# davlee1972/upscale_video

Measured on AMD Instinct MI355X. Metric: frames/sec 1080p->2x Compact (SRVGGNetCompact per-frame SR hot path), higher is better.
Workload: dtype f16 operands / f32 accumulate; 1 GPU; 2x_compact_1080p; tile_size=960, frames_per_call=1

## Files before the change

### upscale_video_amd/csrc/uva_api.hip

```cpp
#include "../../include/uva.h"
#include "uva_denoise.hip.h"
#include "uva_denoise16.hip.h"
#include "uva_generic.hip.h"
#include "uva_kernels.hip.h"
#include "uva_model.h"
#include "uva_pixfmt.h"
#include "uva_plan.h"
#include "uva_repeat.h"
#include "uva_crop.h"
#include "uva_resize.h"
#include "uva_png.hip.h"
#include "uva_wino.h"
#include "uva_sub5.h"
#include "uva_sub10.h"

namespace uva {
int png_read_bgr(const uint8_t* file, size_t len, uint8_t* out, size_t cap, int* h_out, int* w_out, std::string& err);
int png_read_bgr16(const uint8_t* file, size_t len, uint16_t* out, size_t cap, int* h_out, int* w_out, std::string& err);
int zlib_decompress_exact(const uint8_t* in, size_t n, uint8_t* out, size_t out_len, std::string& err);
}

#include <hip/hip_runtime.h>

#include <algorithm>
// ... 264 lines not shown
template <typename T>
int upload(T** dst, const void* src, size_t bytes, hipStream_t st)
{
    HIP_TRY(hipMalloc((void**)dst, bytes));
    HIP_TRY(hipMemcpyAsync(*dst, src, bytes, hipMemcpyHostToDevice, st));
    return 0;
}


template <int NF, int MODE, int R>
int launch_conv_t(uva_net* n, const ConvArgs& a)
{
    const size_t lds = conv_lds_bytes<NF>(MODE == 0 ? 0 : R);
    auto kfn = conv3x3_kernel<NF, MODE, R>;
    if (!n->attr_set[MODE]) {
        HIP_TRY(hipFuncSetAttribute((const void*)kfn, hipFuncAttributeMaxDynamicSharedMemorySize, (int)lds));
        n->attr_set[MODE] = true;
    }
    const int per_cu = NF == 24 ? 2 : 1;
    const int grid = std::max(8, (n->ncu / 8) * 8) * per_cu;
    hipLaunchKernelGGL(kfn, dim3(grid), dim3(256), lds, n->stream, a);
    HIP_TRY(hipGetLastError());
    return 0;
}

template <int ABL>
int launch_trunk64_t(uva_net* n, const ConvArgs& a)
{
    const size_t lds = trunk_lds_bytes<64>();
    auto kfn = trunk_kernel<64, ABL>;
    constexpr int SLOT = 3 + (ABL == 0 ? 0 : ABL == 1 ? 1 : ABL == 2 ? 2 : 3);
    if (!n->attr_set[SLOT]) {
        HIP_TRY(hipFuncSetAttribute((const void*)kfn, hipFuncAttributeMaxDynamicSharedMemorySize, (int)lds));
        n->attr_set[SLOT] = true;
    }
    const int grid = std::max(8, (n->ncu / 8) * 8);
    hipLaunchKernelGGL(kfn, dim3(grid), dim3(512), lds, n->stream, a);
    HIP_TRY(hipGetLastError());
    return 0;
}

int launch_trunk64(uva_net* n, const ConvArgs& a, int ablate = 0)
{
#ifdef UVA_INSTRUMENT
    if (ablate == 1) return launch_trunk64_t<1>(n, a);
    if (ablate == 2) return launch_trunk64_t<2>(n, a);
    if (ablate == 4) return launch_trunk64_t<4>(n, a);
#endif
    (void)ablate;
    return launch_trunk64_t<0>(n, a);
}

template <int NF>
int launch_conv_nf(uva_net* n, int mode, int r, const ConvArgs& a)
{
    if (mode == 0) return launch_conv_t<NF, 0, 1>(n, a);
    if (mode == 1) {
        if (r == 1) return launch_conv_t<NF, 1, 1>(n, a);
        if (r == 2) return launch_conv_t<NF, 1, 2>(n, a);
        if (r == 4) return launch_conv_t<NF, 1, 4>(n, a);
    } else {
        if (r == 1) return launch_conv_t<NF, 2, 1>(n, a);
        if (r == 2) return launch_conv_t<NF, 2, 2>(n, a);
        if (r == 4) return launch_conv_t<NF, 2, 4>(n, a);
    }
    return fail("no kernel for this scale");
}

int launch_conv(uva_net* n, int mode, const ConvArgs& a)
{
    if (n->g.nf == 64) return launch_conv_nf<64>(n, mode, n->g.scale, a);
    if (n->g.nf == 24) return launch_conv_nf<24>(n, mode, n->g.scale, a);
    return fail("no kernel for this trunk width");
}

bool has_tail64(const uva_net* n) { return n->g.nf == 64 && (n->g.scale == 2 || n->g.scale == 4) && n->layers.back().wpk16; }

int launch_tail_u8(uva_net* n, const Workspace* ws, ConvArgs ca, bool u16 = false)
{
    if (has_tail64(n)) {
        const bool x4 = n->g.scale == 4;
        size_t lds;
        void (*kfn)(ConvArgs);
        if (u16) {
            lds = x4 ? tail4_lds_bytes<64, uint16_t>() : tail_lds_bytes<64, uint16_t>();
            kfn = x4 ? tail4_kernel<64, uint16_t> : tail_kernel<64, 2, uint16_t>;
        } else {
            lds = x4 ? tail4_lds_bytes<64>() : tail_lds_bytes<64>();
            kfn = x4 ? tail4_kernel<64, uint8_t> : tail_kernel<64, 2, uint8_t>;
        }
        const int slot = u16 ? 10 : 7;
        if (!n->attr_set[slot]) {
            HIP_TRY(hipFuncSetAttribute((const void*)kfn, hipFuncAttributeMaxDynamicSharedMemorySize, (int)lds));
            n->attr_set[slot] = true;
        }
        const int grid = std::max(8, (n->ncu / 8) * 8);
        const int per_launch = 8 * (2 * (grid / 8)) * ((TAIL_SCHED_MAX - TRUNK_LOOKAHEAD) / 2 - 1);
        ca.sched4 = ws->d_sched4;
        ca.wpk = n->layers.back().wpk16;
        for (int base = 0; base < ws->ntiles4; base += per_launch) {
            ca.tile_base = base;
            ca.ntiles = std::min(per_launch, ws->ntiles4 - base);
            ca.tiles_per_xcd = (ca.ntiles + 7) / 8;
            hipLaunchKernelGGL(kfn, dim3(grid), dim3(512), lds, n->stream, ca);
            HIP_TRY(hipGetLastError());
        }
        return 0;
    }
    if (u16) return fail("the 16-bit route has no tail for this net");
    return launch_conv(n, 1, ca);
}

int launch_trunk(uva_net* n, const Workspace* ws, ConvArgs ca, int ablate = 0)
{
    if (n->g.nf == 64) {
        const int grid = std::max(8, (n->ncu / 8) * 8);
        const int per_launch = 8 * (2 * (grid / 8)) * ((TRUNK_SCHED_MAX - TRUNK_LOOKAHEAD) / 2 - 1);
        ca.sched4 = ws->d_sched4;
        for (int base = 0; base < ws->ntiles4; base += per_launch) {
            ca.tile_base = base;
            ca.ntiles = std::min(per_launch, ws->ntiles4 - base);
            ca.tiles_per_xcd = (ca.ntiles + 7) / 8;
            if (launch_trunk64(n, ca, ablate)) return 1;
        }
        return 0;
    }
    ca.ntiles = ws->ntiles;
    ca.tiles_per_xcd = (ws->ntiles + 7) / 8;
    return launch_conv(n, 0, ca);
}

int launch_trunk2(uva_net* n, const Workspace* ws, const Trunk2Args& a)
{
    const size_t lds = trunk2_lds_bytes<64>();
    auto kfn = trunk2_kernel<64>;
    if (!n->attr_set[8]) {
        HIP_TRY(hipFuncSetAttribute((const void*)kfn, hipFuncAttributeMaxDynamicSharedMemorySize, (int)lds));
        n->attr_set[8] = true;
    }
    hipLaunchKernelGGL(kfn, dim3(ws->grid2), dim3(512), lds, n->stream, a);
    HIP_TRY(hipGetLastError());
    return 0;
}

int launch_trunkw(uva_net* n, const Workspace* ws, TrunkwArgs& a, int i, bool in_negated = false, bool carry_out = false)
{
    for (int k = 0; k < 2; ++k) {
        a.wpk[k] = n->layers[i + k].wpk_w;
        a.bias[k] = n->act16 ? n->layers[i + k].bias_w : n->layers[i + k].bias;
        a.slope[k] = n->layers[i + k].slope;
    }
    if (in_negated) a.wpk[0] = n->layers[i].wpk_wn;
    const int act = !n->act16 ? TW_ACT_F32 : (n->layers[i + 1].flip_w && !carry_out) ? TW_ACT_F16_FLIP : TW_ACT_F16;
    HIP_TRY(launch_trunkw_kernel(n->stream, ws->grid2, a, act));
    return 0;
}

int launch_sub5(uva_net* n, Workspace* ws, const void* src, size_t src_stride, void* dst, size_t dst_stride,
                unsigned long long* dbg = nullptr, int dbg_part = -1)
{
    if (ws->sub5_unfit) return 2;
    if (!ws->d_rows5) {
        std::vector<uint4> rows;
        std::vector<int> nrows;
        ws->grid5 = std::max(8, (n->ncu / 8) * 8);
        std::string err;
        const int rc = build_sub5_rows(ws->h, ws->w, ws->grid5, rows, nrows, &ws->max_rows5, err);
        if (rc == 1) return fail(err);
        if (rc) {
            ws->sub5_unfit = true;
            return 2;
        }
        char* d_mid = nullptr;
        uint4* d_rows = nullptr;
        int* d_nrows = nullptr;
        hipError_t e = hipMalloc((void**)&d_mid, (size_t)ws->h * ws->w * S5_MIDB);
        if (e == hipSuccess) e = hipMalloc((void**)&d_rows, rows.size() * sizeof(uint4));
        if (e == hipSuccess) e = hipMalloc((void**)&d_nrows, nrows.size() * sizeof(int));
        if (e == hipSuccess) e = hipMemcpyAsync(d_rows, rows.data(), rows.size() * sizeof(uint4), hipMemcpyHostToDevice, n->stream);
        if (e == hipSuccess) e = hipMemcpyAsync(d_nrows, nrows.data(), nrows.size() * sizeof(int), hipMemcpyHostToDevice, n->stream);
        if (e == hipSuccess) e = hipStreamSynchronize(n->stream);
        if (e != hipSuccess) {
            if (d_mid) (void)hipFree(d_mid);
            if (d_rows) (void)hipFree(d_rows);
            if (d_nrows) (void)hipFree(d_nrows);
            return fail(std::string("sub5 workspace: ") + hipGetErrorString(e));
        }
        ws->d_mid5 = d_mid; ws->d_rows5 = d_rows; ws->d_nrows5 = d_nrows;
    }
    for (int part = 0; part < 2; ++part) {
        Sub5Args a;
        std::memset(&a, 0, sizeof a);
        a.src = (const uint8_t*)src; a.src_stride = src_stride;
        a.dst = (uint8_t*)dst; a.dst_stride = dst_stride;
        a.mid = ws->d_mid5;
        a.h = ws->h; a.w = ws->w;
        a.rows = ws->d_rows5; a.nrows = ws->d_nrows5; a.max_rows = ws->max_rows5;
        a.dbg = part == dbg_part ? dbg : nullptr;
        for (int i = 0; i < S5_NL; ++i) {
            a.wpk[i] = n->layers[S5_NL * part + i].wpk_s10;
            a.bias[i] = n->layers[S5_NL * part + i].bias_s10;
            a.slope[i] = n->layers[S5_NL * part + i].slope;
        }
        HIP_TRY(launch_sub5_kernel(n->stream, ws->grid5, a, part));
    }
    return 0;
}

int ensure_sub10_rows(uva_net* n, Workspace* ws, int frames)
{
    if (ws->sub10_unfit || frames < 1 || frames > ws->sub10_max_batch) return 2;
    const int bi = frames - 1;
    if (!ws->d_rows10[bi]) {
        std::vector<uint4> rows;
        std::vector<int> nrows;
        ws->grid10 = std::max(8, (n->ncu / 8) * 8);
        std::string err;
        const int rc = build_sub10_rows(ws->h, ws->w, frames, ws->grid10, rows, nrows, &ws->max_rows10[bi], err);
        if (rc == 1) return fail(err);
        if (rc) {
            if (frames == 1) ws->sub10_unfit = true;
            ws->sub10_max_batch = frames - 1;
            return 2;
        }
        uint4* d_rows = nullptr;
        int* d_nrows = nullptr;
        hipError_t e = hipMalloc((void**)&d_rows, rows.size() * sizeof(uint4));
        if (e == hipSuccess) e = hipMalloc((void**)&d_nrows, nrows.size() * sizeof(int));
        if (e == hipSuccess) e = hipMemcpyAsync(d_rows, rows.data(), rows.size() * sizeof(uint4), hipMemcpyHostToDevice, n->stream);
        if (e == hipSuccess) e = hipMemcpyAsync(d_nrows, nrows.data(), nrows.size() * sizeof(int), hipMemcpyHostToDevice, n->stream);
        if (e == hipSuccess) e = hipStreamSynchronize(n->stream);
        if (e != hipSuccess) {
            if (d_rows) (void)hipFree(d_rows);
            if (d_nrows) (void)hipFree(d_nrows);
            return fail(std::string("sub10 row table: ") + hipGetErrorString(e));
        }
        ws->d_rows10[bi] = d_rows;
        ws->d_nrows10[bi] = d_nrows;
    }
    return 0;
}

int launch_sub10(uva_net* n, Workspace* ws, const void* const* srcs, size_t src_stride, void* const* dsts, size_t dst_stride, int frames,
                 unsigned long long* dbg = nullptr)
{
    if (const int rc = ensure_sub10_rows(n, ws, frames)) return rc;
    const int bi = frames - 1;
    Sub10Args a;
    std::memset(&a, 0, sizeof a);
    for (int f = 0; f < S10_MAXB; ++f) {
        a.src[f] = (const uint8_t*)srcs[std::min(f, frames - 1)];
        a.dst[f] = (uint8_t*)dsts[std::min(f, frames - 1)];
    }
    a.src_stride = src_stride;
    a.dst_stride = dst_stride;
    a.h = ws->h; a.w = ws->w;
    a.rows = ws->d_rows10[bi]; a.nrows = ws->d_nrows10[bi]; a.max_rows = ws->max_rows10[bi];
    a.dbg = dbg;
    for (int i = 0; i < S10_NL; ++i) {
        a.wpk[i] = n->layers[i].wpk_s10;
        a.bias[i] = n->layers[i].bias_s10;
        a.slope[i] = n->layers[i].slope;
    }
    HIP_TRY(launch_sub10_kernel(n->stream, ws->grid10, a));
    return 0;
}
int launch_sub10(uva_net* n, Workspace* ws, const void* src, size_t src_stride, void* dst, size_t dst_stride, unsigned long long* dbg = nullptr)
{
    return launch_sub10(n, ws, &src, src_stride, &dst, dst_stride, 1, dbg);
}

bool is_sub10_net(const uva_net* n)
{
    return !n->generic && n->g.nf == 24 && n->g.scale == 1 && (int)n->g.convs.size() == S10_NL;
}

int launch_pair24(uva_net* n, const ConvArgs& a)
{
    const size_t lds = pair24_lds_bytes();
    if (!n->attr_set[9]) {
        HIP_TRY(hipFuncSetAttribute((const void*)pair24_kernel, hipFuncAttributeMaxDynamicSharedMemorySize, (int)lds));
        n->attr_set[9] = true;
    }
    const int grid = std::max(8, (n->ncu / 8) * 8) * 2;
    hipLaunchKernelGGL(pair24_kernel, dim3(grid), dim3(256), lds, n->stream, a);
    HIP_TRY(hipGetLastError());
    return 0;
}

int launch_head(uva_net* n, bool f32, const HeadArgs& a, bool u16 = false)
{
    if (u16) {
        if (n->g.nf != 64 || !a.sink) return fail("the 16-bit route has no head for this net");
        const dim3 grid(std::min(a.ntiles, n->ncu * HEADP_WG_PER_CU)), block(256);
        hipLaunchKernelGGL((headp_kernel<64, 2>), grid, block, headp_lds_bytes<64>(), n->stream, a);
        HIP_TRY(hipGetLastError());
        return 0;
    }
    const char* const hp = uva::debug_env("UVA_HEAD_PERSIST");
    const bool persist = !hp || std::atoi(hp) != 0;
    if (persist && a.sink) {
        const dim3 grid(std::min(a.ntiles, n->ncu * HEADP_WG_PER_CU)), block(256);
        if (n->g.nf == 64) {
            const size_t lds = headp_lds_bytes<64>();
            if (f32) hipLaunchKernelGGL((headp_kernel<64, 1>), grid, block, lds, n->stream, a);
            else hipLaunchKernelGGL((headp_kernel<64, 0>), grid, block, lds, n->stream, a);
        } else {
// ... 3323 lines not shown
```

### upscale_video_amd/csrc/uva_wino.h

```cpp
#pragma once
#include <hip/hip_runtime.h>
#include <stdint.h>

#include "uva_plan.h"

namespace uva {

struct TrunkwArgs {
    const char* in_act;
    char* out_act;
    const void* wpk[2];
    const float* bias[2];
    const float* slope[2];
    const Trunk2Step* steps;
    const int* nsteps;
    int max_steps;
    _Float16* sink;
    unsigned long long* dbg;
};

enum { TW_ACT_F32 = 0, TW_ACT_F16 = 1, TW_ACT_F16_FLIP = 2 };

hipError_t launch_trunkw_kernel(hipStream_t stream, int grid, const TrunkwArgs& a, int act);

}
```

### upscale_video_amd/csrc/uva_wino.hip

```cpp
#include <atomic>

#include "uva_wino.hip.h"

namespace uva {

template <int ACT>
static hipError_t launch_act(hipStream_t stream, int grid, const TrunkwArgs& a)
{
    auto kfn = trunkw_kernel<64, ACT>;
    static std::atomic<bool> attr_done[64];
    int dev = 0;
    hipError_t e = hipGetDevice(&dev);
    if (e != hipSuccess) return e;
    if (dev < 0 || dev >= 64 || !attr_done[dev].load(std::memory_order_acquire)) {
        e = hipFuncSetAttribute((const void*)kfn, hipFuncAttributeMaxDynamicSharedMemorySize, (int)TW_LDS_BYTES);
        if (e != hipSuccess) return e;
        if (dev >= 0 && dev < 64) attr_done[dev].store(true, std::memory_order_release);
    }
    hipLaunchKernelGGL(kfn, dim3(grid), dim3(512), TW_LDS_BYTES, stream, a);
    return hipGetLastError();
}

hipError_t launch_trunkw_kernel(hipStream_t stream, int grid, const TrunkwArgs& a, int act)
{
    switch (act) {
    case TW_ACT_F32: return launch_act<TW_ACT_F32>(stream, grid, a);
    case TW_ACT_F16: return launch_act<TW_ACT_F16>(stream, grid, a);
    case TW_ACT_F16_FLIP: return launch_act<TW_ACT_F16_FLIP>(stream, grid, a);
    }
    return hipErrorInvalidValue;
}

}
```

### upscale_video_amd/csrc/uva_wino.hip.h

```cpp
#pragma once
#include <type_traits>

#include "uva_devutil.hip.h"
#include "uva_wino.h"

namespace uva {

constexpr int TW_AROWB = 4 * 2 * 16 * 64;
constexpr int TW_BROWB = 4 * 2 * 15 * 64;
constexpr int TW_AROWS = 6, TW_BROWS = 10;
constexpr int TW_RAWROWB = 34 * 128;
constexpr int TW_RAWSLOTB = 4 * TW_RAWROWB;
constexpr int TW_RAW_PIECES = TW_RAWSLOTB / 1024;
constexpr int TW_ARING = 0;
constexpr int TW_BRING = TW_ARING + TW_AROWS * TW_AROWB;
constexpr int TW_RAW = TW_BRING + TW_BROWS * TW_BROWB;
constexpr int TW_PRM = TW_RAW + 2 * TW_RAWSLOTB;
constexpr int TW_FLAGS_OFF = TW_PRM + 2 * PARAM_LDS + 64;
constexpr int TW_LDS_BYTES = TW_FLAGS_OFF + 16;
static_assert(TW_RAW_PIECES == 17 && TW_RAWSLOTB % 1024 == 0, "raw slot = whole LDS-DMA pieces");
static_assert(TW_LDS_BYTES <= 160 * 1024, "trunkw kernel LDS budget");
static_assert(TW_RAW % 128 == 0 && TW_RAWROWB % 128 == 0, "raw pixel records are 128-byte aligned (the octet XOR flips address bits 4..6)");


__device__ __forceinline__ unsigned tw_piece_const(int i, int wave, int lane)
{
    const int q = (4 * i + wave) * 64 + lane;
    const int r = q / 272, u = q - r * 272;
    const int rec = u >> 3, sl = u & 7;
    const int par = rec >= 17 ? 1 : 0, h = rec - 17 * par;
    return (unsigned)((r << 13) | ((2 * h + par) * 128 + ((sl ^ (h & 7)) << 4)));
}

__device__ __forceinline__ unsigned dpp_row_shl1(unsigned v)
{
    return (unsigned)__builtin_amdgcn_mov_dpp((int)v, 0x101, 0xf, 0xf, true);
}
__device__ __forceinline__ unsigned pk_add_f16(unsigned a, unsigned b)
{
    return __builtin_bit_cast(unsigned, (half2v)(__builtin_bit_cast(half2v, a) + __builtin_bit_cast(half2v, b)));
}

#define TW_PRIO_K 2
#define TW_PRIO_E 0
#define TW_PRIO_KA TW_PRIO_K
#define TW_PRIO_EA TW_PRIO_E
#define TW_PRIO_KB TW_PRIO_K
#define TW_PRIO_EB TW_PRIO_E

#ifdef UVA_INSTRUMENT
#define TW_STAMP(k) do { if (stamp) a.dbg[16 * it + 8 * grp + (k)] = __builtin_amdgcn_s_memtime(); } while (0)
#else
#define TW_STAMP(k) do { } while (0)
#endif

template <int NF, int ACT>
__global__ __launch_bounds__(512, 2) UVA_NO_PK_F32 void trunkw_kernel(TrunkwArgs a)
{
    static_assert(NF == 64, "written for 64 features");
    constexpr int PIXB = 128;
    constexpr int TW_PFF = 12;
    constexpr int TW_PFF_B = 6;
    constexpr int TW_RAW_F0 = 4, TW_RAW_GAP = 12, TW_RAW_STRIDE = 3;
    constexpr int TW_DMA_PIECES = 5;
    constexpr int PFF_A = TW_PFF;

    extern __shared__ __attribute__((aligned(16))) char smem[];
    const unsigned lds0 = lds_offset(smem);
    float* const prm_all = (float*)(smem + TW_PRM);

    const int wave8 = __builtin_amdgcn_readfirstlane(threadIdx.x >> 6);
    const int grp = wave8 >> 2;
    const int wave = wave8 & 3;
    const int lane = threadIdx.x & 63;

#ifdef UVA_INSTRUMENT
    const unsigned long long t_entry = __builtin_amdgcn_s_memtime();
#endif
    const Trunk2Step* const steps = a.steps + (size_t)blockIdx.x * (a.max_steps + TW_PAD_STEPS);
    auto load_a = [&](int g) __attribute__((always_inline)) { return scalar_load16(&steps[g].a); };
    auto load_b = [&](int g) __attribute__((always_inline)) { return scalar_load16(&steps[g].b); };
    const uint4 e_first = load_a(0), e_second = load_a(1);
    const int nsteps = __builtin_amdgcn_readfirstlane(a.nsteps[blockIdx.x]);
    if (nsteps <= 0) return;
#ifdef UVA_INSTRUMENT
    const bool stamp = a.dbg != nullptr && blockIdx.x == 0 && (threadIdx.x & 255) == 0;
    if (stamp && grp == 0) a.dbg[16 * (nsteps + 2)] = t_entry;
#endif

    float prm_b = 0.f, prm_s = 0.f;
    if (wave == 0) {
        prm_b = (grp ? a.bias[1] : a.bias[0])[lane];
        prm_s = (grp ? a.slope[1] : a.slope[0])[lane];
    }
    half8 w[24];
    {
        const half8* wp = (const half8*)(grp ? a.wpk[1] : a.wpk[0]);
#pragma unroll
        for (int i = 0; i < 24; ++i) w[i] = wp[(i * 4 + wave) * 64 + lane];
    }
    unsigned dma_pc2[3];
#pragma unroll
    for (int i = 0; i < 3; ++i)
        dma_pc2[i] = tw_piece_const(2 * i, wave, lane) | (2 * i + 1 < 5 ? tw_piece_const(2 * i + 1, wave, lane) << 16 : 0u);
    auto issue_rows = [&](const uint4 e, int slot, auto i0c, auto i1c) __attribute__((always_inline)) {
        constexpr int I0 = decltype(i0c)::value, I1 = decltype(i1c)::value;
        const unsigned ey = __builtin_amdgcn_readfirstlane(e.y);
        const unsigned lo = __builtin_amdgcn_readfirstlane(e.x), hi = ey & 0xffu;
        const char* base = a.in_act + (((unsigned long long)hi << 32) | lo);
        const int pitch = __builtin_amdgcn_readfirstlane(e.z) & 0xffffff;
        const unsigned fadd = ((ey >> 27) & 1u) ? (unsigned)__builtin_amdgcn_readfirstlane(e.w) : 0u;
#pragma unroll
        for (int i = I0; i < I1; ++i) {
            if (4 * i + wave >= TW_RAW_PIECES) continue;
            const unsigned pc = (dma_pc2[i >> 1] >> (16 * (i & 1))) & 0xffffu;
            unsigned off = __umul24(pc >> 13, (unsigned)pitch) + (pc & 0x1fffu);
            if (fadd) off += (pc & 0x1800u) ? fadd : 0u;
            glds16_s(base, off, lds0 + TW_RAW + slot * TW_RAWSLOTB + (4 * i + wave) * 1024);
        }
    };

    auto vlane_of = [](int l) __attribute__((always_inline)) { const int p_ = l & 15, o_ = l >> 4; return (unsigned)(p_ * 64 + ((o_ ^ ((p_ >> 1) & 3)) << 4)); };

    const unsigned vlane_c = vlane_of(lane);
    const unsigned t_lo = (unsigned)((lane & 15) * PIXB + (((lane >> 4) ^ (lane & 7)) << 4));
    const unsigned t_hi = (unsigned)(((lane & 15) + 1) * PIXB + (((lane >> 4) ^ (((lane & 15) + 1) & 7)) << 4));
    auto transform_row = [&](const char* rrow, int pos) __attribute__((always_inline)) {
        const unsigned a_lo = t_lo, a_hi = t_hi;
        char* const vrow = smem + TW_ARING + pos * TW_AROWB + vlane_c;
        half8 d[2][4];
#pragma unroll
        for (int t = 0; t < 2; ++t) {
            d[t][0] = *(const half8*)(rrow + (a_lo ^ (t ? 64u : 0u)));
            d[t][1] = *(const half8*)(rrow + (a_lo ^ (t ? 64u : 0u)) + 17 * PIXB);
            d[t][2] = *(const half8*)(rrow + (a_hi ^ (t ? 64u : 0u)));
            d[t][3] = *(const half8*)(rrow + (a_hi ^ (t ? 64u : 0u)) + 17 * PIXB);
        }
#pragma unroll
        for (int t = 0; t < 2; ++t) {
            *(half8*)(vrow + 0 * 2048 + t * 1024) = pk_sub(d[t][0], d[t][2]);
            *(half8*)(vrow + 1 * 2048 + t * 1024) = d[t][1] + d[t][2];
            *(half8*)(vrow + 2 * 2048 + t * 1024) = pk_sub(d[t][2], d[t][1]);
            *(half8*)(vrow + 3 * 2048 + t * 1024) = pk_sub(d[t][1], d[t][3]);
        }
    };

    auto transform_half = [&](const char* rrow, int pos, int t) __attribute__((always_inline)) {
        const unsigned a_lo = t_lo ^ (t ? 64u : 0u), a_hi = t_hi ^ (t ? 64u : 0u);
        char* const vrow = smem + TW_ARING + pos * TW_AROWB + vlane_c + t * 1024;
        const half8 d0 = *(const half8*)(rrow + a_lo), d1 = *(const half8*)(rrow + a_lo + 17 * PIXB);
        const half8 d2 = *(const half8*)(rrow + a_hi), d3 = *(const half8*)(rrow + a_hi + 17 * PIXB);
        *(half8*)(vrow + 0 * 2048) = pk_sub(d0, d2);
        *(half8*)(vrow + 1 * 2048) = d1 + d2;
        *(half8*)(vrow + 2 * 2048) = pk_sub(d2, d1);
        *(half8*)(vrow + 3 * 2048) = pk_sub(d1, d3);
    };

    auto transform_rows = [&](int slot, int pos0) __attribute__((always_inline)) {
        int pos = pos0 + wave;
        pos = pos >= TW_AROWS ? pos - TW_AROWS : pos;
        transform_row(smem + TW_RAW + slot * TW_RAWSLOTB + wave * TW_RAWROWB, pos);
    };

    const bool six = (__builtin_amdgcn_readfirstlane(e_first.y) >> 25) & 1u;
    if (grp == 0) {
        issue_rows(e_first, 0, std::integral_constant<int, 0>{}, std::integral_constant<int, 5>{});
        issue_rows(e_second, 1, std::integral_constant<int, 0>{}, std::integral_constant<int, 5>{});
        if (six && wave < 2) {
            const unsigned lo = __builtin_amdgcn_readfirstlane(e_first.x), hi = __builtin_amdgcn_readfirstlane(e_first.y) & 0xffu;
            const int pitch = __builtin_amdgcn_readfirstlane(e_first.z) & 0xffffff;
            const char* base = a.in_act + (((unsigned long long)hi << 32) | lo) - (size_t)(2 - wave) * pitch;
#pragma unroll
            for (int i = 0; i < 5; ++i) {
                int q = i * 64 + lane;
                q = q < 272 ? q : 271;
                const int rec = q >> 3, sl = q & 7, par = rec >= 17 ? 1 : 0, hh = rec - 17 * par;
                glds16_s(base, (unsigned)((2 * hh + par) * 128 + ((sl ^ (hh & 7)) << 4)), lds0 + TW_BRING + wave * 5120 + i * 1024);
            }
        }
#pragma unroll
        for (int i = 0; i < 24; ++i) asm volatile("" : "+v"(w[i]));
        asm volatile("s_waitcnt vmcnt(0)" ::: "memory");
    }
    if (wave == 0) {
        float* prm = prm_all + grp * (PARAM_LDS / 4);
        prm[lane] = prm_b;
        prm[64 + lane] = prm_s;
        prm[128 + lane] = prm_s <= 1.f ? __builtin_inff() : -__builtin_inff();
    }
    group_barrier();
    if (grp == 1) {
        transform_rows(0, 2);
        if (six && wave < 2) transform_row(smem + TW_BRING + wave * 5120, wave);
    }
    group_barrier();

    const float* const bias_lds = prm_all + grp * (PARAM_LDS / 4);
    const float* const prm_lds = bias_lds + 64;
    const f32x4 zero4 = {0.f, 0.f, 0.f, 0.f};
    const f32x4 bias4 = *(const f32x4*)(bias_lds + 16 * wave + 4 * (lane >> 4));
    const f32x4 s4 = *(const f32x4*)(prm_lds + 16 * wave + 4 * (lane >> 4));
    const f32x4 i4 = *(const f32x4*)(prm_lds + 64 + 16 * wave + 4 * (lane >> 4));

    f32x4 acc[4][4];
    [[maybe_unused]] auto prefetch = [&](auto ring_tag, int base_pos, auto& pre) __attribute__((always_inline)) {
        constexpr bool BR = decltype(ring_tag)::value;
        constexpr int ROWB = BR ? TW_BROWB : TW_AROWB;
        constexpr int PFF = BR ? TW_PFF_B : PFF_A;
        static_assert(PFF <= 8, "the fragments read ahead of the barrier are window row 0's");
        const unsigned r0 = vlane_c + (unsigned)((BR ? TW_BRING : TW_ARING) + base_pos * ROWB);
#pragma unroll
        for (int f = 0; f < PFF; ++f) pre[f] = *(const half8*)(smem + r0 + (f & 3) * (ROWB / 4) + ((f >> 2) & 1) * (ROWB / 8));
    };
    auto kloop = [&](auto ring_tag, int base_pos, auto&& slice, auto&& hook, [[maybe_unused]] const auto& pre) __attribute__((always_inline)) {
        constexpr bool BR = decltype(ring_tag)::value;
        constexpr int INR = 0;
        constexpr int ROWB = BR ? TW_BROWB : TW_AROWB, NROWS = BR ? TW_BROWS : TW_AROWS;
        constexpr int JS = ROWB / 4, CS = ROWB / 8;
        constexpr int PFF = BR ? TW_PFF_B : PFF_A;
        constexpr int NFRAG = 48, RQ = PFF + 1;
        unsigned radr[6];
        const unsigned vlane = vlane_c;
#pragma unroll
        for (int R = 0; R < 6; ++R) {
            int pos = base_pos + R;
            pos = pos >= NROWS ? pos - NROWS : pos;
            radr[R] = vlane + (unsigned)((BR ? TW_BRING : TW_ARING) + pos * ROWB);
        }
        auto read_f = [&](int f) __attribute__((always_inline)) -> half8 {
            const int R = f >> 3, ch = (f >> 2) & 1, j = f & 3;
            return *(const half8*)(smem + radr[R] + j * JS + ch * CS);
        };
        half8 bq[RQ];
        __builtin_amdgcn_sched_barrier(0);
#pragma unroll
        for (int f = 0; f < PFF; ++f) {
            if constexpr (BR) bq[f] = pre[f];
            else bq[f] = read_f(f);
        }
        __builtin_amdgcn_sched_barrier(0);
        static_for<NFRAG>([&](auto fc) __attribute__((always_inline)) {
            constexpr int f = decltype(fc)::value;
            if constexpr (f + PFF < NFRAG) bq[(f + PFF) % RQ] = read_f(f + PFF);
            constexpr int R = f >> 3, ch = (f >> 2) & 1, j = f & 3;
            const half8 b = bq[f % RQ];
            static_for<4>([&](auto nc) __attribute__((always_inline)) {
                constexpr int n = decltype(nc)::value, dy = R - n;
                if constexpr (dy >= 0 && dy <= 2) {
                    constexpr bool first = dy == 0 && ch == 0;
                    acc[n][j] = __builtin_amdgcn_mfma_f32_16x16x32_f16(w[(j * 3 + dy) * 2 + ch], b, first ? (j == 1 ? bias4 : zero4) : acc[n][j], 0, 0, 0);
                }
            });
            if constexpr (R >= 3 && R - 3 < INR) slice(std::integral_constant<int, R - 3>{}, std::integral_constant<int, (f & 7)>{});
            hook(fc);
            __builtin_amdgcn_sched_barrier(0);
        });
    };

    struct RowSt {
        f32x2 u, v;
        unsigned x0, x1, y0, y1;
        unsigned t[4], q[8];
    };
    f32x2 neg1 = {-1.f, -1.f};
    asm volatile("" : "+v"(neg1));
    auto fin_sum = [&](RowSt& st, int n, int hh) __attribute__((always_inline)) {
        const f32x2 m0 = {acc[n][0][2 * hh], acc[n][0][2 * hh + 1]}, m1 = {acc[n][1][2 * hh], acc[n][1][2 * hh + 1]};
        const f32x2 m2 = {acc[n][2][2 * hh], acc[n][2][2 * hh + 1]}, m3 = {acc[n][3][2 * hh], acc[n][3][2 * hh + 1]};
        st.u = (m0 + m1) + m2;
        st.v = __builtin_elementwise_fma(m3, neg1, __builtin_elementwise_fma(m2, neg1, m1));
    };
    const half2v s16v[2] = {half2v{(_Float16)s4[0], (_Float16)s4[1]}, half2v{(_Float16)s4[2], (_Float16)s4[3]}};
    auto fin_act = [&](RowSt& st, int hh) __attribute__((always_inline)) {
        if constexpr (ACT != TW_ACT_F32) {
            const half2v hu = __builtin_convertvector(st.u, half2v), hv = __builtin_convertvector(st.v, half2v);
            const half2v mu = hu * s16v[hh], mv = hv * s16v[hh];
            const unsigned xu = __builtin_bit_cast(unsigned, __builtin_elementwise_max(hu, mu));
            const unsigned xv = __builtin_bit_cast(unsigned, __builtin_elementwise_max(hv, mv));
            if (hh == 0) { st.x0 = xu; st.y0 = xv; } else { st.x1 = xu; st.y1 = xv; }
            return;
        }
        const f32x2 sl = {s4[2 * hh], s4[2 * hh + 1]};
        const f32x2 us = st.u * sl, vs = st.v * sl;
        const f32x2 pu = {__builtin_amdgcn_fmed3f(st.u[0], us[0], i4[2 * hh]), __builtin_amdgcn_fmed3f(st.u[1], us[1], i4[2 * hh + 1])};
        const f32x2 pv = {__builtin_amdgcn_fmed3f(st.v[0], vs[0], i4[2 * hh]), __builtin_amdgcn_fmed3f(st.v[1], vs[1], i4[2 * hh + 1])};
        const unsigned xu = __builtin_bit_cast(unsigned, __builtin_convertvector(pu, half2v));
        const unsigned xv = __builtin_bit_cast(unsigned, __builtin_convertvector(pv, half2v));
        if (hh == 0) { st.x0 = xu; st.y0 = xv; } else { st.x1 = xu; st.y1 = xv; }
    };

    const int niter = nsteps + 2;
    __builtin_amdgcn_s_waitcnt(0x0f70);
    RowSt st2[2];
    if (grp == 0) {
        uint4 e_own = load_a(0);
        int a6 = 0;
        int b10 = 0;
        const int cg = lane >> 4, p = lane & 15;
        const int oo = 2 * (wave & 1) + (cg >> 1);
        const unsigned wlane = p < 15 ? (unsigned)(TW_BRING + (2 * (cg & 1)) * (TW_BROWB / 4) + (wave >> 1) * (TW_BROWB / 8) + p * 64 +
                                                    ((oo ^ ((p >> 1) & 3)) << 4))
                                      : (unsigned)(TW_FLAGS_OFF - 64 + 16 * cg);
        const unsigned w64 = (unsigned)(TW_BRING + (wave >> 1) * (TW_BROWB / 8) + p * 64 + ((oo ^ ((p >> 1) & 3)) << 4) + 8 * (cg & 1));
        const unsigned wrow = p < 15 ? (unsigned)TW_BROWB : 0u;
        const unsigned wj = p < 15 ? (unsigned)(TW_BROWB / 4) : 0u;
        half8 pre[PFF_A];
        for (int it = 0; it < niter; ++it) {
            TW_STAMP(0);
            const unsigned ey = __builtin_amdgcn_readfirstlane(e_own.y);
            int rmask = 15, b10w = b10;
            bool in0 = true, in1 = true, edge = false;
            auto set_step = [&](const unsigned eyv, const int b10v) __attribute__((always_inline)) {
                const int c_lo = (eyv >> 12) & 63, c_hi = (eyv >> 18) & 63;
                rmask = (eyv >> 8) & 15;
                const int pm = ((eyv >> 27) & 1u) ? (p & 7) : p;
                in0 = 2 * pm >= c_lo && 2 * pm < c_hi;
                in1 = 2 * pm + 1 >= c_lo && 2 * pm + 1 < c_hi;
                edge = rmask != 15 || c_lo != 0 || c_hi != 32;
                b10w = b10v;
            };
            auto slice = [&](RowSt& st, auto edge_tag, auto nc, auto kc) __attribute__((always_inline)) {
                constexpr int n = decltype(nc)::value, k = decltype(kc)::value;
                if constexpr (k == 0) fin_sum(st, n, 0);
                else if constexpr (k == 1) fin_act(st, 0);
                else if constexpr (k == 2) fin_sum(st, n, 1);
                else if constexpr (k == 3) fin_act(st, 1);
                else if constexpr (k == 4) {
                    if constexpr (decltype(edge_tag)::value) {
                        const bool rin = (rmask >> n) & 1;
                        const unsigned k0 = (rin && in0) ? 0xffffffffu : 0u, k1 = (rin && in1) ? 0xffffffffu : 0u;
                        st.x0 &= k0; st.x1 &= k0;
                        st.y0 &= k1; st.y1 &= k1;
                    }
                    st.t[0] = dpp_row_shl1(st.x0); st.t[1] = dpp_row_shl1(st.x1);
                    st.t[2] = dpp_row_shl1(st.y0); st.t[3] = dpp_row_shl1(st.y1);
                } else if constexpr (k == 5) {
                    st.q[0] = pk_sub_f16(st.x0, st.t[0]); st.q[1] = pk_sub_f16(st.x1, st.t[1]);
                    st.q[2] = pk_add_f16(st.y0, st.t[0]); st.q[3] = pk_add_f16(st.y1, st.t[1]);
                    st.q[4] = pk_sub_f16(st.t[0], st.y0); st.q[5] = pk_sub_f16(st.t[1], st.y1);
                    st.q[6] = pk_sub_f16(st.y0, st.t[2]); st.q[7] = pk_sub_f16(st.y1, st.t[3]);
                } else if constexpr (k == 6) {
                    int pos = b10w + n;
                    pos = pos >= TW_BROWS ? pos - TW_BROWS : pos;
                    if (p < 15) {
                        char* const w0 = smem + w64 + (unsigned)pos * TW_BROWB;
#pragma unroll
                        for (int j = 0; j < 4; ++j) *(uint2*)(w0 + j * (TW_BROWB / 4)) = make_uint2(st.q[2 * j], st.q[2 * j + 1]);
                    }
                } else if constexpr (k == 7) {
                } else if constexpr (k == 8) {
                    const auto s02a = __builtin_amdgcn_permlane16_swap(st.q[0], st.q[4], false, false);
                    const auto s02b = __builtin_amdgcn_permlane16_swap(st.q[1], st.q[5], false, false);
                    const auto s13a = __builtin_amdgcn_permlane16_swap(st.q[2], st.q[6], false, false);
                    const auto s13b = __builtin_amdgcn_permlane16_swap(st.q[3], st.q[7], false, false);
                    st.q[0] = s02a[0]; st.q[1] = s02b[0]; st.q[2] = s02a[1]; st.q[3] = s02b[1];
                    st.q[4] = s13a[0]; st.q[5] = s13b[0]; st.q[6] = s13a[1]; st.q[7] = s13b[1];
                } else {
                    int pos = b10w + n;
                    pos = pos >= TW_BROWS ? pos - TW_BROWS : pos;
                    char* const w0 = smem + wlane + (unsigned)pos * wrow;
                    *(uint4*)w0 = make_uint4(st.q[0], st.q[1], st.q[2], st.q[3]);
                    *(uint4*)(w0 + wj) = make_uint4(st.q[4], st.q[5], st.q[6], st.q[7]);
                }
            };
            set_step(ey, b10);
            if (it < nsteps) {
                __builtin_amdgcn_s_setprio(TW_PRIO_KA);
                auto no_hook = [](auto) __attribute__((always_inline)) {};
                kloop(std::false_type{}, a6, [&](auto nc, auto kc) __attribute__((always_inline)) { slice(st2[0], std::false_type{}, nc, kc); }, no_hook, pre);
                __builtin_amdgcn_s_setprio(TW_PRIO_EA);
            }
            TW_STAMP(1);
            group_barrier();
            TW_STAMP(2);
            if (it < nsteps) {
                auto rest = [&](auto edge_tag) __attribute__((always_inline)) {
                    static_for<2>([&](auto rc) __attribute__((always_inline)) {
                        static_for<8>([&](auto kc) __attribute__((always_inline)) {
                            slice(st2[0], edge_tag, std::integral_constant<int, 2 * decltype(rc)::value>{}, kc);
                            slice(st2[1], edge_tag, std::integral_constant<int, 2 * decltype(rc)::value + 1>{}, kc);
                        });
                    });
                };
                if (edge) rest(std::true_type{}); else rest(std::false_type{});
            }
            e_own = load_a(it + 1 < nsteps ? it + 1 : nsteps - 1);
            TW_STAMP(3);
            a6 = a6 + 4 >= TW_AROWS ? a6 + 4 - TW_AROWS : a6 + 4;
            group_barrier();
            b10 = b10 + 4 >= TW_BROWS ? b10 + 4 - TW_BROWS : b10 + 4;
        }
    } else {
        int a6 = 0, b10 = 0;
        uint4 e_k = make_uint4(0, 0, 0, 0), e_3 = make_uint4(0, 0, 0, 0);
        const int cg = lane >> 4, p = lane & 15;
        const int col = 2 * p + (cg & 1);
        const unsigned olane = (unsigned)(col * PIXB + 32 * wave + 16 * (cg >> 1));
        char* const sink = (char*)a.sink + lane * PIXB;
        const unsigned flip0 = (s4[0] > 1.f ? 0x8000u : 0u) | (s4[1] > 1.f ? 0x80000000u : 0u);
        const unsigned flip1 = (s4[2] > 1.f ? 0x8000u : 0u) | (s4[3] > 1.f ? 0x80000000u : 0u);
        auto make_slice = [&](const uint4 e) __attribute__((always_inline)) {
            const unsigned ey = __builtin_amdgcn_readfirstlane(e.y), lo = __builtin_amdgcn_readfirstlane(e.x);
            const size_t off = ((unsigned long long)(ey & 0xffu) << 32) | lo;
            const int pitch = __builtin_amdgcn_readfirstlane(e.z) & 0xffffff;
            const int vy = (ey >> 8) & 7, vx = (ey >> 11) & 63, v0 = (ey >> 17) & 7;
            const bool fold = (ey >> 25) & 1u;
            const unsigned fadd = fold ? (unsigned)__builtin_amdgcn_readfirstlane(e.w) : 0u;
            char* const obase = a.out_act + off + olane + ((fold && p >= 8) ? fadd : 0u);
            const bool colok = (fold ? (col & 15) : col) < vx;
            return [&, obase, pitch, vy, v0, colok](RowSt& st, auto nc, auto kc) __attribute__((always_inline)) {
                constexpr int n = decltype(nc)::value, k = decltype(kc)::value;
                if constexpr (k == 0) fin_sum(st, n, 0);
                else if constexpr (k == 1) fin_act(st, 0);
                else if constexpr (k == 2) fin_sum(st, n, 1);
                else if constexpr (k == 3) fin_act(st, 1);
                else if constexpr (k == 4) {
                    if constexpr (ACT == TW_ACT_F16_FLIP) {
                        st.x0 ^= flip0; st.y0 ^= flip0;
                        st.x1 ^= flip1; st.y1 ^= flip1;
                    }
                    const auto x = __builtin_amdgcn_permlane16_swap(st.x0, st.y0, false, false);
                    const auto y = __builtin_amdgcn_permlane16_swap(st.x1, st.y1, false, false);
                    st.q[0] = x[0]; st.q[1] = y[0]; st.q[2] = x[1]; st.q[3] = y[1];
                } else if constexpr (k == 5) {
                    char* dst = (n >= v0 && n < vy && colok) ? obase + (size_t)n * pitch : sink;
                    *(uint4*)dst = make_uint4(st.q[0], st.q[1], st.q[2], st.q[3]);
                }
            };
        };
        uint4 e_dma = load_a(2 <= nsteps + TW_PAD_STEPS - 1 ? 2 : nsteps + TW_PAD_STEPS - 1);
        unsigned st_prev = 0;
        for (int it = 0; it < niter; ++it) {
            TW_STAMP(0);
            issue_rows(e_dma, it & 1, std::integral_constant<int, 0>{}, std::integral_constant<int, TW_DMA_PIECES>{});
            e_dma = load_a(it + 3 <= nsteps + TW_PAD_STEPS - 1 ? it + 3 : nsteps + TW_PAD_STEPS - 1);
            const unsigned st_cur = (unsigned)__builtin_amdgcn_readfirstlane((int)(it >= 2 ? (__builtin_amdgcn_readfirstlane(e_3.y) >> 24) & 1u : 0u));
            if (it >= 2 && ((__builtin_amdgcn_readfirstlane(e_3.y) >> 24) & 1u)) {
                auto sl3 = make_slice(e_3);
                static_for<2>([&](auto rc) __attribute__((always_inline)) {
                    static_for<6>([&](auto kc) __attribute__((always_inline)) {
                        sl3(st2[0], std::integral_constant<int, 2 * decltype(rc)::value>{}, kc);
                        sl3(st2[1], std::integral_constant<int, 2 * decltype(rc)::value + 1>{}, kc);
                    });
                });
            }
            e_k = load_b(it >= 1 ? it - 1 : 0);
            const unsigned kact = (it >= 1 && it <= nsteps) ? (__builtin_amdgcn_readfirstlane(e_k.y) >> 24) & 1u : 0u;
            int bp = b10 - 4 - 2;
            bp = bp < 0 ? bp + TW_BROWS : bp;
            half8 pre[TW_PFF_B];
            TW_STAMP(1);
#ifdef UVA_INSTRUMENT
            asm volatile("s_waitcnt vmcnt(0)" ::: "memory");
            st_prev = st_cur;
#else
            {
                constexpr int P0 = TW_DMA_PIECES, P = TW_DMA_PIECES - 1;
                const unsigned nst = st_prev + st_cur;
                if (wave == 0) {
                    if (nst == 2) asm volatile("s_waitcnt vmcnt(%0)" ::"n"(P0 + 8) : "memory");
                    else if (nst == 1) asm volatile("s_waitcnt vmcnt(%0)" ::"n"(P0 + 4) : "memory");
                    else asm volatile("s_waitcnt vmcnt(%0)" ::"n"(P0) : "memory");
                } else {
                    if (nst == 2) asm volatile("s_waitcnt vmcnt(%0)" ::"n"(P + 8) : "memory");
                    else if (nst == 1) asm volatile("s_waitcnt vmcnt(%0)" ::"n"(P + 4) : "memory");
                    else asm volatile("s_waitcnt vmcnt(%0)" ::"n"(P) : "memory");
                }
                st_prev = st_cur;
            }
#endif
            prefetch(std::true_type{}, bp, pre);
            asm volatile("s_barrier" ::: "memory");
            TW_STAMP(2);
            [[maybe_unused]] auto raw_rows = [&]() __attribute__((always_inline)) {
                if (it + 1 < nsteps) {
                    int pos0 = a6 + 4 + 2;
                    pos0 = pos0 >= TW_AROWS ? pos0 - TW_AROWS : pos0;
                    transform_rows((it + 1) & 1, pos0);
                }
            };
            unsigned solo = (unsigned)__builtin_amdgcn_readfirstlane((int)((kact ^ 1u) & (it + 1 < nsteps ? 1u : 0u)));
            asm volatile("" : "+s"(solo));
            if (solo) {
                int pos = a6 + 4 + 2 + wave;
                pos = pos >= 2 * TW_AROWS ? pos - 2 * TW_AROWS : pos >= TW_AROWS ? pos - TW_AROWS : pos;
                const char* const rr = smem + TW_RAW + ((it + 1) & 1) * TW_RAWSLOTB + wave * TW_RAWROWB;
                transform_half(rr, pos, 0);
                __builtin_amdgcn_sched_barrier(0);
                transform_half(rr, pos, 1);
            }
            TW_STAMP(4);
            if (kact) {
                __builtin_amdgcn_s_setprio(TW_PRIO_KB);
                auto slk = make_slice(e_k);
                int rpos = a6 + 4 + 2 + wave;
                rpos = rpos >= 2 * TW_AROWS ? rpos - 2 * TW_AROWS : rpos >= TW_AROWS ? rpos - TW_AROWS : rpos;
                const char* const rrow = smem + TW_RAW + ((it + 1) & 1) * TW_RAWSLOTB + wave * TW_RAWROWB;
                char* const vrow = smem + TW_ARING + rpos * TW_AROWB + vlane_c;
                half8 rd[4];
                auto raw_hook = [&](auto fc) __attribute__((always_inline)) {
                    constexpr int f = decltype(fc)::value;
                    constexpr int H1 = TW_RAW_F0 + TW_RAW_GAP + 3 * TW_RAW_STRIDE + 1;
                    static_assert(H1 + TW_RAW_GAP + 3 * TW_RAW_STRIDE < 48, "the transform ends inside the k-loop");
                    constexpr int t = f >= H1 ? 1 : 0, g = f - (t ? H1 : TW_RAW_F0);
                    const unsigned a_lo = t_lo ^ (t ? 64u : 0u), a_hi = t_hi ^ (t ? 64u : 0u);
                    if constexpr (g == 0) {
                        rd[0] = *(const half8*)(rrow + a_lo); rd[1] = *(const half8*)(rrow + a_lo + 17 * PIXB);
                        rd[2] = *(const half8*)(rrow + a_hi); rd[3] = *(const half8*)(rrow + a_hi + 17 * PIXB);
                    } else if constexpr (g == TW_RAW_GAP) *(half8*)(vrow + 0 * 2048 + t * 1024) = pk_sub(rd[0], rd[2]);
                    else if constexpr (g == TW_RAW_GAP + TW_RAW_STRIDE) *(half8*)(vrow + 3 * 2048 + t * 1024) = pk_sub(rd[1], rd[3]);
                    else if constexpr (g == TW_RAW_GAP + 2 * TW_RAW_STRIDE) *(half8*)(vrow + 1 * 2048 + t * 1024) = rd[1] + rd[2];
                    else if constexpr (g == TW_RAW_GAP + 3 * TW_RAW_STRIDE) *(half8*)(vrow + 2 * 2048 + t * 1024) = pk_sub(rd[2], rd[1]);
                };
                kloop(std::true_type{}, bp, [&](auto nc, auto kc) __attribute__((always_inline)) { slk(st2[0], nc, kc); }, raw_hook, pre);
                __builtin_amdgcn_s_setprio(TW_PRIO_EB);
            }
            e_3 = e_k;
            TW_STAMP(3);
            group_barrier();
            a6 = a6 + 4 >= TW_AROWS ? a6 + 4 - TW_AROWS : a6 + 4;
            b10 = b10 + 4 >= TW_BROWS ? b10 + 4 - TW_BROWS : b10 + 4;
        }
    }
    asm volatile("s_waitcnt vmcnt(0)" ::: "memory");
}

}
```

Before: 505.6 frames/s.

## Carry partial row accumulators across steps in Winograd trunk kernel

Adds a CARRY variant of the fused two-layer Winograd trunk kernel. Instead of re-reading two overlapping halo rows from a 6-row A-ring each step, it keeps partial sums for the next step's first output rows in two extra accumulator sets, so the A-ring shrinks to 4 rows and each step does fewer MFMAs on halo rows. It adds register pressure (6x4 accumulators instead of 4x4) and a separate carry-in path for the first step, and shortens the A-ring prefetch depth. The variant is picked at launch by the net's carry flag, which defaults to true.

Result: faster. 512.7 frames/s (median of 6 runs) (+1.4%).

```diff
diff --git a/upscale_video_amd/csrc/uva_api.hip b/upscale_video_amd/csrc/uva_api.hip
--- a/upscale_video_amd/csrc/uva_api.hip
+++ b/upscale_video_amd/csrc/uva_api.hip
@@ -440,7 +440,7 @@
     }
     if (in_negated) a.wpk[0] = n->layers[i].wpk_wn;
     const int act = !n->act16 ? TW_ACT_F32 : (n->layers[i + 1].flip_w && !carry_out) ? TW_ACT_F16_FLIP : TW_ACT_F16;
-    HIP_TRY(launch_trunkw_kernel(n->stream, ws->grid2, a, act));
+    HIP_TRY(launch_trunkw_kernel(n->stream, ws->grid2, a, act, n->carry));
     return 0;
 }
 
diff --git a/upscale_video_amd/csrc/uva_wino.h b/upscale_video_amd/csrc/uva_wino.h
--- a/upscale_video_amd/csrc/uva_wino.h
+++ b/upscale_video_amd/csrc/uva_wino.h
@@ -21,6 +21,6 @@
 
 enum { TW_ACT_F32 = 0, TW_ACT_F16 = 1, TW_ACT_F16_FLIP = 2 };
 
-hipError_t launch_trunkw_kernel(hipStream_t stream, int grid, const TrunkwArgs& a, int act);
+hipError_t launch_trunkw_kernel(hipStream_t stream, int grid, const TrunkwArgs& a, int act, bool row_carry = true);
 
 }
diff --git a/upscale_video_amd/csrc/uva_wino.hip b/upscale_video_amd/csrc/uva_wino.hip
--- a/upscale_video_amd/csrc/uva_wino.hip
+++ b/upscale_video_amd/csrc/uva_wino.hip
@@ -4,10 +4,11 @@
 
 namespace uva {
 
-template <int ACT>
+template <int ACT, bool CARRY>
 static hipError_t launch_act(hipStream_t stream, int grid, const TrunkwArgs& a)
 {
-    auto kfn = trunkw_kernel<64, ACT>;
+    auto kfn = trunkw_kernel<64, ACT, CARRY>;
+    constexpr int TW_LDS_BYTES = TwLds<CARRY>::BYTES;
     static std::atomic<bool> attr_done[64];
     int dev = 0;
     hipError_t e = hipGetDevice(&dev);
@@ -21,14 +22,20 @@
     return hipGetLastError();
 }
 
-hipError_t launch_trunkw_kernel(hipStream_t stream, int grid, const TrunkwArgs& a, int act)
+template <bool CARRY>
+static hipError_t launch_carry(hipStream_t stream, int grid, const TrunkwArgs& a, int act)
 {
     switch (act) {
-    case TW_ACT_F32: return launch_act<TW_ACT_F32>(stream, grid, a);
-    case TW_ACT_F16: return launch_act<TW_ACT_F16>(stream, grid, a);
-    case TW_ACT_F16_FLIP: return launch_act<TW_ACT_F16_FLIP>(stream, grid, a);
+    case TW_ACT_F32: return launch_act<TW_ACT_F32, CARRY>(stream, grid, a);
+    case TW_ACT_F16: return launch_act<TW_ACT_F16, CARRY>(stream, grid, a);
+    case TW_ACT_F16_FLIP: return launch_act<TW_ACT_F16_FLIP, CARRY>(stream, grid, a);
     }
     return hipErrorInvalidValue;
 }
 
+hipError_t launch_trunkw_kernel(hipStream_t stream, int grid, const TrunkwArgs& a, int act, bool row_carry)
+{
+    return row_carry ? launch_carry<true>(stream, grid, a, act) : launch_carry<false>(stream, grid, a, act);
 }
+
+}
diff --git a/upscale_video_amd/csrc/uva_wino.hip.h b/upscale_video_amd/csrc/uva_wino.hip.h
--- a/upscale_video_amd/csrc/uva_wino.hip.h
+++ b/upscale_video_amd/csrc/uva_wino.hip.h
@@ -8,19 +8,27 @@
 
 constexpr int TW_AROWB = 4 * 2 * 16 * 64;
 constexpr int TW_BROWB = 4 * 2 * 15 * 64;
-constexpr int TW_AROWS = 6, TW_BROWS = 10;
+constexpr int TW_BROWS = 10;
 constexpr int TW_RAWROWB = 34 * 128;
 constexpr int TW_RAWSLOTB = 4 * TW_RAWROWB;
 constexpr int TW_RAW_PIECES = TW_RAWSLOTB / 1024;
-constexpr int TW_ARING = 0;
-constexpr int TW_BRING = TW_ARING + TW_AROWS * TW_AROWB;
-constexpr int TW_RAW = TW_BRING + TW_BROWS * TW_BROWB;
-constexpr int TW_PRM = TW_RAW + 2 * TW_RAWSLOTB;
-constexpr int TW_FLAGS_OFF = TW_PRM + 2 * PARAM_LDS + 64;
-constexpr int TW_LDS_BYTES = TW_FLAGS_OFF + 16;
+template <bool CARRY>
+struct TwLds {
+    static constexpr int AROWS = CARRY ? 4 : 6;
+    static constexpr int ARING = 0;
+    static constexpr int BRING = ARING + AROWS * TW_AROWB;
+    static constexpr int RAW = BRING + TW_BROWS * TW_BROWB;
+    static constexpr int PRM = RAW + 2 * TW_RAWSLOTB;
+    static constexpr int FLAGS_OFF = PRM + 2 * PARAM_LDS + 64;
+    static constexpr int BYTES = FLAGS_OFF + 16;
+    static constexpr int SIX_RAW = BRING, SIX_RAWB = 5120, SIX_ROWS = BRING + 16384;
+    static_assert(BYTES <= 160 * 1024, "trunkw kernel LDS budget");
+    static_assert(RAW % 128 == 0 && TW_RAWROWB % 128 == 0, "raw pixel records are 128-byte aligned (the octet XOR flips address bits 4..6)");
+    static_assert(2 * SIX_RAWB <= 16384 && SIX_ROWS + 2 * TW_AROWB <= RAW, "the first step's extra rows fit the B-ring");
+    static_assert((AROWS - 1) * TW_AROWB + 3 * (TW_AROWB / 4) + TW_AROWB / 8 < 65536, "a ring row's fragments are immediate offsets of one address");
+};
 static_assert(TW_RAW_PIECES == 17 && TW_RAWSLOTB % 1024 == 0, "raw slot = whole LDS-DMA pieces");
-static_assert(TW_LDS_BYTES <= 160 * 1024, "trunkw kernel LDS budget");
-static_assert(TW_RAW % 128 == 0 && TW_RAWROWB % 128 == 0, "raw pixel records are 128-byte aligned (the octet XOR flips address bits 4..6)");
+static_assert(TwLds<true>::BYTES + 16384 == TwLds<false>::BYTES, "the carry frees two A-ring rows (left unused)");
 
 
 __device__ __forceinline__ unsigned tw_piece_const(int i, int wave, int lane)
@@ -54,12 +62,14 @@
 #define TW_STAMP(k) do { } while (0)
 #endif
 
-template <int NF, int ACT>
+template <int NF, int ACT, bool CARRY = true>
 __global__ __launch_bounds__(512, 2) UVA_NO_PK_F32 void trunkw_kernel(TrunkwArgs a)
 {
     static_assert(NF == 64, "written for 64 features");
     constexpr int PIXB = 128;
-    constexpr int TW_PFF = 12;
+    using Lds = TwLds<CARRY>;
+    constexpr int TW_AROWS = Lds::AROWS, TW_ARING = Lds::ARING, TW_BRING = Lds::BRING, TW_RAW = Lds::RAW, TW_PRM = Lds::PRM, TW_FLAGS_OFF = Lds::FLAGS_OFF;
+    constexpr int TW_PFF = CARRY ? 6 : 12;
     constexpr int TW_PFF_B = 6;
     constexpr int TW_RAW_F0 = 4, TW_RAW_GAP = 12, TW_RAW_STRIDE = 3;
     constexpr int TW_DMA_PIECES = 5;
@@ -125,9 +135,9 @@
     const unsigned vlane_c = vlane_of(lane);
     const unsigned t_lo = (unsigned)((lane & 15) * PIXB + (((lane >> 4) ^ (lane & 7)) << 4));
     const unsigned t_hi = (unsigned)(((lane & 15) + 1) * PIXB + (((lane >> 4) ^ (((lane & 15) + 1) & 7)) << 4));
-    auto transform_row = [&](const char* rrow, int pos) __attribute__((always_inline)) {
+    auto transform_row = [&](const char* rrow, int vbase) __attribute__((always_inline)) {
         const unsigned a_lo = t_lo, a_hi = t_hi;
-        char* const vrow = smem + TW_ARING + pos * TW_AROWB + vlane_c;
+        char* const vrow = smem + vbase + vlane_c;
         half8 d[2][4];
 #pragma unroll
         for (int t = 0; t < 2; ++t) {
@@ -159,7 +169,7 @@
     auto transform_rows = [&](int slot, int pos0) __attribute__((always_inline)) {
         int pos = pos0 + wave;
         pos = pos >= TW_AROWS ? pos - TW_AROWS : pos;
-        transform_row(smem + TW_RAW + slot * TW_RAWSLOTB + wave * TW_RAWROWB, pos);
+        transform_row(smem + TW_RAW + slot * TW_RAWSLOTB + wave * TW_RAWROWB, TW_ARING + pos * TW_AROWB);
     };
 
     const bool six = (__builtin_amdgcn_readfirstlane(e_first.y) >> 25) & 1u;
@@ -175,7 +185,7 @@
                 int q = i * 64 + lane;
                 q = q < 272 ? q : 271;
                 const int rec = q >> 3, sl = q & 7, par = rec >= 17 ? 1 : 0, hh = rec - 17 * par;
-                glds16_s(base, (unsigned)((2 * hh + par) * 128 + ((sl ^ (hh & 7)) << 4)), lds0 + TW_BRING + wave * 5120 + i * 1024);
+                glds16_s(base, (unsigned)((2 * hh + par) * 128 + ((sl ^ (hh & 7)) << 4)), lds0 + Lds::SIX_RAW + wave * Lds::SIX_RAWB + i * 1024);
             }
         }
 #pragma unroll
@@ -190,8 +200,8 @@
     }
     group_barrier();
     if (grp == 1) {
-        transform_rows(0, 2);
-        if (six && wave < 2) transform_row(smem + TW_BRING + wave * 5120, wave);
+        transform_rows(0, CARRY ? 0 : 2);
+        if (six && wave < 2) transform_row(smem + Lds::SIX_RAW + wave * Lds::SIX_RAWB, CARRY ? Lds::SIX_ROWS + wave * TW_AROWB : TW_ARING + wave * TW_AROWB);
     }
     group_barrier();
 
@@ -202,7 +212,7 @@
     const f32x4 s4 = *(const f32x4*)(prm_lds + 16 * wave + 4 * (lane >> 4));
     const f32x4 i4 = *(const f32x4*)(prm_lds + 64 + 16 * wave + 4 * (lane >> 4));
 
-    f32x4 acc[4][4];
+    f32x4 acc[CARRY ? 6 : 4][4];
     [[maybe_unused]] auto prefetch = [&](auto ring_tag, int base_pos, auto& pre) __attribute__((always_inline)) {
         constexpr bool BR = decltype(ring_tag)::value;
         constexpr int ROWB = BR ? TW_BROWB : TW_AROWB;
@@ -257,6 +267,61 @@
         });
     };
 
+    [[maybe_unused]] auto kloop_carry = [&]() __attribute__((always_inline)) {
+        if constexpr (CARRY) {
+        constexpr int JS = TW_AROWB / 4, CS = TW_AROWB / 8;
+        constexpr int PFF = PFF_A, NFRAG = 32, RQ = PFF + 1;
+        const char* const r0 = smem + TW_ARING + vlane_c;
+        auto read_f = [&](int f) __attribute__((always_inline)) -> half8 {
+            return *(const half8*)(r0 + (f >> 3) * TW_AROWB + (f & 3) * JS + ((f >> 2) & 1) * CS);
+        };
+        half8 bq[RQ];
+        __builtin_amdgcn_sched_barrier(0);
+#pragma unroll
+        for (int f = 0; f < PFF; ++f) bq[f] = read_f(f);
+        __builtin_amdgcn_sched_barrier(0);
+        static_for<NFRAG>([&](auto fc) __attribute__((always_inline)) {
+            constexpr int f = decltype(fc)::value;
+            if constexpr (f + PFF < NFRAG) bq[(f + PFF) % RQ] = read_f(f + PFF);
+            constexpr int R = (f >> 3) + 2, ch = (f >> 2) & 1, j = f & 3;
+            const half8 b = bq[f % RQ];
+            static_for<6>([&](auto nc) __attribute__((always_inline)) {
+                constexpr int n = decltype(nc)::value, dy = R - n;
+                if constexpr (dy >= 0 && dy <= 2) {
+                    constexpr bool first = dy == 0 && ch == 0;
+                    constexpr bool handed = R == 2 && ch == 0 && n < 2;
+                    acc[n][j] = __builtin_amdgcn_mfma_f32_16x16x32_f16(w[(j * 3 + dy) * 2 + ch], b,
+                                                                       first ? (j == 1 ? bias4 : zero4) : acc[handed ? n + 4 : n][j], 0, 0, 0);
+                }
+            });
+            __builtin_amdgcn_sched_barrier(0);
+        });
+        }
+    };
+    [[maybe_unused]] auto carry_in = [&]() __attribute__((always_inline)) {
+        if constexpr (CARRY) {
+        constexpr int JS = TW_AROWB / 4, CS = TW_AROWB / 8;
+        const char* const r0 = smem + Lds::SIX_ROWS + vlane_c;
+        static_for<2>([&](auto rc) __attribute__((always_inline)) {
+            constexpr int R = decltype(rc)::value;
+            half8 b[8];
+#pragma unroll
+            for (int f = 0; f < 8; ++f) b[f] = *(const half8*)(r0 + R * TW_AROWB + (f & 3) * JS + (f >> 2) * CS);
+            static_for<8>([&](auto fc) __attribute__((always_inline)) {
+                constexpr int ch = decltype(fc)::value >> 2, j = decltype(fc)::value & 3;
+                static_for<2>([&](auto nc) __attribute__((always_inline)) {
+                    constexpr int n = decltype(nc)::value, dy = R - n;
+                    if constexpr (dy >= 0) {
+                        constexpr bool first = dy == 0 && ch == 0;
+                        acc[n + 4][j] = __builtin_amdgcn_mfma_f32_16x16x32_f16(w[(j * 3 + dy) * 2 + ch], b[decltype(fc)::value],
+                                                                               first ? (j == 1 ? bias4 : zero4) : acc[n + 4][j], 0, 0, 0);
+                    }
+                });
+            });
+        });
+        }
+    };
+
     struct RowSt {
         f32x2 u, v;
         unsigned x0, x1, y0, y1;
@@ -294,8 +359,13 @@
     RowSt st2[2];
     if (grp == 0) {
         uint4 e_own = load_a(0);
-        int a6 = 0;
+        [[maybe_unused]] int a6 = 0;
         int b10 = 0;
+        if constexpr (CARRY) {
+#pragma unroll
+            for (int j = 0; j < 4; ++j) acc[4][j] = acc[5][j] = zero4;
+            if (six) carry_in();
+        }
         const int cg = lane >> 4, p = lane & 15;
         const int oo = 2 * (wave & 1) + (cg >> 1);
         const unsigned wlane = p < 15 ? (unsigned)(TW_BRING + (2 * (cg & 1)) * (TW_BROWB / 4) + (wave >> 1) * (TW_BROWB / 8) + p * 64 +
@@ -304,7 +374,7 @@
         const unsigned w64 = (unsigned)(TW_BRING + (wave >> 1) * (TW_BROWB / 8) + p * 64 + ((oo ^ ((p >> 1) & 3)) << 4) + 8 * (cg & 1));
         const unsigned wrow = p < 15 ? (unsigned)TW_BROWB : 0u;
         const unsigned wj = p < 15 ? (unsigned)(TW_BROWB / 4) : 0u;
-        half8 pre[PFF_A];
+        [[maybe_unused]] half8 pre[PFF_A];
         for (int it = 0; it < niter; ++it) {
             TW_STAMP(0);
             const unsigned ey = __builtin_amdgcn_readfirstlane(e_own.y);
@@ -367,7 +437,8 @@
             if (it < nsteps) {
                 __builtin_amdgcn_s_setprio(TW_PRIO_KA);
                 auto no_hook = [](auto) __attribute__((always_inline)) {};
-                kloop(std::false_type{}, a6, [&](auto nc, auto kc) __attribute__((always_inline)) { slice(st2[0], std::false_type{}, nc, kc); }, no_hook, pre);
+                if constexpr (CARRY) kloop_carry();
+                else kloop(std::false_type{}, a6, [&](auto nc, auto kc) __attribute__((always_inline)) { slice(st2[0], std::false_type{}, nc, kc); }, no_hook, pre);
                 __builtin_amdgcn_s_setprio(TW_PRIO_EA);
             }
             TW_STAMP(1);
@@ -386,7 +457,7 @@
             }
             e_own = load_a(it + 1 < nsteps ? it + 1 : nsteps - 1);
             TW_STAMP(3);
-            a6 = a6 + 4 >= TW_AROWS ? a6 + 4 - TW_AROWS : a6 + 4;
+            if constexpr (!CARRY) a6 = a6 + 4 >= TW_AROWS ? a6 + 4 - TW_AROWS : a6 + 4;
             group_barrier();
             b10 = b10 + 4 >= TW_BROWS ? b10 + 4 - TW_BROWS : b10 + 4;
         }
@@ -474,7 +545,7 @@
             TW_STAMP(2);
             [[maybe_unused]] auto raw_rows = [&]() __attribute__((always_inline)) {
                 if (it + 1 < nsteps) {
-                    int pos0 = a6 + 4 + 2;
+                    int pos0 = CARRY ? 0 : a6 + 4 + 2;
                     pos0 = pos0 >= TW_AROWS ? pos0 - TW_AROWS : pos0;
                     transform_rows((it + 1) & 1, pos0);
                 }
@@ -482,7 +553,7 @@
             unsigned solo = (unsigned)__builtin_amdgcn_readfirstlane((int)((kact ^ 1u) & (it + 1 < nsteps ? 1u : 0u)));
             asm volatile("" : "+s"(solo));
             if (solo) {
-                int pos = a6 + 4 + 2 + wave;
+                int pos = CARRY ? wave : a6 + 4 + 2 + wave;
                 pos = pos >= 2 * TW_AROWS ? pos - 2 * TW_AROWS : pos >= TW_AROWS ? pos - TW_AROWS : pos;
                 const char* const rr = smem + TW_RAW + ((it + 1) & 1) * TW_RAWSLOTB + wave * TW_RAWROWB;
                 transform_half(rr, pos, 0);
@@ -493,7 +564,7 @@
             if (kact) {
                 __builtin_amdgcn_s_setprio(TW_PRIO_KB);
                 auto slk = make_slice(e_k);
-                int rpos = a6 + 4 + 2 + wave;
+                int rpos = CARRY ? wave : a6 + 4 + 2 + wave;
                 rpos = rpos >= 2 * TW_AROWS ? rpos - 2 * TW_AROWS : rpos >= TW_AROWS ? rpos - TW_AROWS : rpos;
                 const char* const rrow = smem + TW_RAW + ((it + 1) & 1) * TW_RAWSLOTB + wave * TW_RAWROWB;
                 char* const vrow = smem + TW_ARING + rpos * TW_AROWB + vlane_c;
@@ -518,7 +589,7 @@
             e_3 = e_k;
             TW_STAMP(3);
             group_barrier();
-            a6 = a6 + 4 >= TW_AROWS ? a6 + 4 - TW_AROWS : a6 + 4;
+            if constexpr (!CARRY) a6 = a6 + 4 >= TW_AROWS ? a6 + 4 - TW_AROWS : a6 + 4;
             b10 = b10 + 4 >= TW_BROWS ? b10 + 4 - TW_BROWS : b10 + 4;
         }
     }
```
